# andimarafioti/faster-qwen3-tts

Measured on AMD Instinct MI355X. Metric: real-time factor (audio s / wall s), Qwen3-TTS-12Hz-0.6B voice-clone streaming chunk_size=8; p50 TTFA in ttfa_ms_p50, higher is better.
Workload: dtype bf16

## Files before the change

### faster-qwen3-tts_amd/csrc/decode_kernels.cuh

```cuda
#pragma once
#include "fq3_common.cuh"
#include <initializer_list>

namespace fq3 {

enum { PRO_PLAIN = 0, PRO_NORM = 1, PRO_COMBINE = 2 };
enum { EPI_STORE = 0, EPI_RESIDUAL = 1, EPI_SWIGLU = 2 };

constexpr int kHeadDim = 128;
constexpr int kKeysPerTile = 64;
constexpr int kMaxWorkers = 8;
constexpr int kPartStride = kHeadDim + 4;


struct GemvArgs {
    const void* W; int N; int K;
    const void* x;
    const void* norm_w; float eps;
    const void* bias;
    void* y;
    const void* res;
    void* xn_out;
    int up_off;
    const float* part; int n_part; int rep;
// ... 244 lines not shown
    const void* x = PRO == PRO_COMBINE ? static_cast<const void*>(a.part) : a.x;
    hipLaunchKernelGGL((gemv_kernel<T, NCH, PRO, EPI, NT, M, R>), dim3(grid), dim3(256), shm, s, a.W, x, a.norm_w, a.N, a.K, a.eps, a.up_off,
                       a.n_part, a.rep, t);
}

struct AttnArgs {
    const void* qkv;
    const void* q_norm_w; const void* k_norm_w; float eps;
    const float* cos_row; const float* sin_row;
    void* kcache; void* vcache; int max_seq;
    const int* table; int blk_stride;
    const int* pos_ptr; int pos_imm; int n_pad;
    const int* done_ptr;
    int n_kv; float* part; float scale;
    int rep; void* out;
};

template <typename T, int REP, bool PAGED>
__device__ __forceinline__ void attn_decode_body(const AttnArgs& a) {
    constexpr int HD = kHeadDim, KS = kKeysPerTile, NG = KS / 16;
    const int g = blockIdx.x, s = blockIdx.y, S = gridDim.y;
    __shared__ float qs[REP][HD];
    __shared__ float knew[HD], vnew[HD];
    __shared__ float wo[4][REP][HD];
    __shared__ float wm[4][REP], wl[4][REP];
    const int tid = threadIdx.x, wave = tid >> 6, lane = tid & 63;
    const int sub = lane >> 4, c = lane & 15;
    const T* qkv = reinterpret_cast<const T*>(a.qkv);
    const int q_dim = a.n_kv * REP * HD, kv_dim = a.n_kv * HD;
    T* kc = reinterpret_cast<T*>(a.kcache) + (PAGED ? (size_t)g * KS * HD : (size_t)g * a.max_seq * HD);
// ... 166 lines not shown
constexpr int kAttnDecodeLeadDwords = 14;
template <typename T, int REP, bool PAGED>
__global__ __launch_bounds__(256) void attn_decode_kernel(const int* table, const void* qkv, void* kcache, void* vcache, const int* pos_ptr,
                                                          int max_seq, int n_kv, int blk_stride, int pos_imm, AttnTail t) {
    AttnArgs a = attn_args_of(t);
    a.table = table; a.qkv = qkv; a.kcache = kcache; a.vcache = vcache; a.pos_ptr = pos_ptr;
    a.max_seq = max_seq; a.n_kv = n_kv; a.blk_stride = blk_stride; a.pos_imm = pos_imm;
    attn_decode_body<T, REP, PAGED>(a);
}
template <typename T, int REP, bool PAGED>
inline void attn_decode_launch(const AttnArgs& a, int workers, hipStream_t s) {
    hipLaunchKernelGGL((attn_decode_kernel<T, REP, PAGED>), dim3(a.n_kv, workers), dim3(256), 0, s, a.table, a.qkv, a.kcache, a.vcache, a.pos_ptr,
                       a.max_seq, a.n_kv, a.blk_stride, a.pos_imm, attn_tail(a));
}

template <typename T>
__device__ __forceinline__ void attn_pred_body(const AttnArgs& a, int head) {
    constexpr int HD = kHeadDim;
    const int g = head / a.rep, hh = head - g * a.rep;
    const int lane = threadIdx.x & 63, sub = lane >> 4, c = lane & 15;
    const int pos = a.pos_imm;
    const T* qkv = reinterpret_cast<const T*>(a.qkv);
    const int q_dim = a.n_kv * a.rep * HD, kv_dim = a.n_kv * HD;
    T* kc = reinterpret_cast<T*>(a.kcache) + (size_t)g * a.max_seq * HD;
    T* vc = reinterpret_cast<T*>(a.vcache) + (size_t)g * a.max_seq * HD;
    Raw8<T> qraw, knraw, vnraw, qwraw, kwraw, kr[4], vr[4];
    ldraw<false>(qraw, qkv + (size_t)head * HD + c * 8);
    ldraw<false>(knraw, qkv + q_dim + (size_t)g * HD + c * 8);
    ldraw<false>(vnraw, qkv + q_dim + kv_dim + (size_t)g * HD + c * 8);
    ldraw<false>(qwraw, reinterpret_cast<const T*>(a.q_norm_w) + c * 8);
    ldraw<false>(kwraw, reinterpret_cast<const T*>(a.k_norm_w) + c * 8);
    const f32x4 cs0 = *reinterpret_cast<const f32x4*>(a.cos_row + ((c * 8) & 63)), cs1 = *reinterpret_cast<const f32x4*>(a.cos_row + ((c * 8 + 4) & 63));
    const f32x4 sn0 = *reinterpret_cast<const f32x4*>(a.sin_row + ((c * 8) & 63)), sn1 = *reinterpret_cast<const f32x4*>(a.sin_row + ((c * 8 + 4) & 63));
#pragma unroll
    for (int i = 0; i < 4; ++i) {
        int key = i * 4 + sub;
        key = key < a.max_seq ? key : a.max_seq - 1;
        ldraw<false>(kr[i], kc + (size_t)key * HD + c * 8);
        ldraw<false>(vr[i], vc + (size_t)key * HD + c * 8);
    }
    __builtin_amdgcn_sched_barrier(0);
    const float sgn = c < 8 ? -1.f : 1.f;
    const float cs[8] = {cs0.x, cs0.y, cs0.z, cs0.w, cs1.x, cs1.y, cs1.z, cs1.w};
    const float sn[8] = {sgn * sn0.x, sgn * sn0.y, sgn * sn0.z, sgn * sn0.w, sgn * sn1.x, sgn * sn1.y, sgn * sn1.z, sgn * sn1.w};
    auto norm_rope = [&](const Raw8<T>& raw, const Raw8<T>& wraw, float (&out)[8]) {
#pragma clang fp contract(off)
        float x[8], w[8];
        unpack(raw, x); unpack(wraw, w);
        float ss = 0.f;
#pragma unroll
        for (int i = 0; i < 8; ++i) ss = fmaf(x[i], x[i], ss);
        ss = row16_sum(ss);
        const float rs = 1.0f / sqrtf(ss / (float)HD + a.eps);
#pragma unroll
        for (int i = 0; i < 8; i += 2) {
            float u = x[i] * rs, v = x[i + 1] * rs;
            DT<T>::rnd2(u, v);
            u *= w[i]; v *= w[i + 1];
            DT<T>::rnd2(u, v);
            x[i] = u; x[i + 1] = v;
        }
#pragma unroll
        for (int i = 0; i < 8; i += 2) {
            float a0 = x[i] * cs[i], a1 = x[i + 1] * cs[i + 1];
            float b0 = row16_xor8(x[i]) * sn[i], b1 = row16_xor8(x[i + 1]) * sn[i + 1];
            DT<T>::rnd2(a0, a1); DT<T>::rnd2(b0, b1);
            float r0 = a0 + b0, r1 = a1 + b1;
            DT<T>::rnd2(r0, r1);
            out[i] = r0; out[i + 1] = r1;
        }
    };
    float qr[8], knew[8], vnew[8];
    norm_rope(qraw, qwraw, qr);
    norm_rope(knraw, kwraw, knew);
    unpack(vnraw, vnew);
    if (hh == 0 && sub == 0) {
        DT<T>::st8(kc + (size_t)pos * HD + c * 8, knew);
        DT<T>::st8(vc + (size_t)pos * HD + c * 8, vnew);
    }
    float sc[5];
#pragma unroll
    for (int i = 0; i < 4; ++i) {
        float kf[8], s = 0.f;
        unpack(kr[i], kf);
#pragma unroll
        for (int d = 0; d < 8; ++d) s = fmaf(qr[d], kf[d], s);
        s = row16_sum(s);
        sc[i] = (i * 4 + sub < pos) ? s * a.scale : -INFINITY;
    }
    {
        float s = 0.f;
#pragma unroll
        for (int d = 0; d < 8; ++d) s = fmaf(qr[d], knew[d], s);
        s = row16_sum(s);
        sc[4] = sub == 0 ? s * a.scale : -INFINITY;
    }
    const float mx = wave_max(fmaxf(fmaxf(fmaxf(sc[0], sc[1]), fmaxf(sc[2], sc[3])), sc[4]));
    float p[5], lsum = 0.f, o[8];
#pragma unroll
    for (int i = 0; i < 5; ++i) { p[i] = __expf(sc[i] - mx); lsum += p[i]; }
    lsum = wave_sum(lsum) * (1.0f / 16.0f);
#pragma unroll
    for (int d = 0; d < 8; ++d) o[d] = p[4] * vnew[d];
#pragma unroll
    for (int i = 0; i < 4; ++i) {
        float vf[8];
        if (!(i * 4 + sub < pos)) zero(vr[i]);
        unpack(vr[i], vf);
#pragma unroll
        for (int d = 0; d < 8; ++d) o[d] = fmaf(p[i], vf[d], o[d]);
    }
    const float inv = 1.0f / lsum;
#pragma unroll
    for (int d = 0; d < 8; ++d) o[d] = xrow_sum(o[d]) * inv;
    if (sub == 0) DT<T>::st8(reinterpret_cast<T*>(a.out) + (size_t)head * HD + c * 8, o);
}

template <typename T>
__device__ __forceinline__ void attn_pred_body(const AttnArgs& a) { attn_pred_body<T>(a, (int)blockIdx.x); }

template <typename T, int REP>
__device__ __forceinline__ void attn_pred_group_body(const AttnArgs& a, int g) {
    constexpr int HD = kHeadDim;
// ... 103 lines not shown
}

constexpr int kAttnPredLeadDwords = 14;
template <typename T>
__global__ __launch_bounds__(64) void attn_pred_kernel(const void* qkv, const void* q_norm_w, const void* k_norm_w, void* kcache, void* vcache,
                                                       int n_kv, int rep, int max_seq, int pos_imm, AttnTail t) {
    AttnArgs a = attn_args_of(t);
    a.qkv = qkv; a.q_norm_w = q_norm_w; a.k_norm_w = k_norm_w; a.kcache = kcache; a.vcache = vcache;
    a.n_kv = n_kv; a.rep = rep; a.max_seq = max_seq; a.pos_imm = pos_imm;
    attn_pred_body<T>(a);
}
template <typename T>
inline void attn_pred_launch(const AttnArgs& a, int heads, hipStream_t s) {
    hipLaunchKernelGGL((attn_pred_kernel<T>), dim3(heads), dim3(64), 0, s, a.qkv, a.q_norm_w, a.k_norm_w, a.kcache, a.vcache,
                       a.n_kv, a.rep, a.max_seq, a.pos_imm, attn_tail(a));
}

template <typename T>
__global__ __launch_bounds__(256) void rmsnorm_kernel(const T* x, const T* w, T* y, int K, float eps) {
    __shared__ float red[8];
    float ss = 0.f;
    for (int e = threadIdx.x; e < K; e += 256) { const float v = DT<T>::ld(x + e); ss = fmaf(v, v, ss); }
    ss = block_sum<4>(ss, red);
    const float rs = 1.0f / sqrtf(ss / (float)K + eps);
    for (int e = threadIdx.x; e < K; e += 256)
        DT<T>::st(y + e, DT<T>::ld(w + e) * DT<T>::rnd(DT<T>::ld(x + e) * rs));
}

template <typename T>
__global__ void copy_kernel(T* dst, const T* src, int n) {
// ... 126 lines not shown
```

### faster-qwen3-tts_amd/csrc/fq3_api.hip

```cpp
#define FQ3_SKINNY_EXTERN
#include "fq3_ctx.h"
#include "sampler.cuh"
#include "sampler_wave.cuh"
#include "skinny_gemm.cuh"

#include <cstdio>
#include <cstdlib>
#include <cstring>
#include <map>
#include <string>
#include <type_traits>
#include <vector>

using namespace fq3;

static thread_local std::string g_err;
static int fail(int code, const std::string& m) { g_err = m; return code; }
int fq3_fail_(int code, const std::string& m) { return fail(code, m); }
#define HIPCHK(x) do { hipError_t e_ = (x); if (e_ != hipSuccess) return fail(FQ3_EHIP, std::string(#x) + ": " + hipGetErrorString(e_)); } while (0)

extern "C" const char* fq3_last_error(void) { return g_err.c_str(); }
extern "C" void fq3_set_error_(const char* msg) { g_err = msg ? msg : ""; }
extern "C" int fq3_abi_version(void) { return FQ3_ABI_VERSION; }

// ... 190 lines not shown
    if ((r = dmalloc(c, &c->qkv2, (size_t)qkvm * c->esz))) return r;
    if ((r = dmalloc(c, &c->attn_out, (size_t)qkvm * c->esz))) return r;
    if ((r = dmalloc(c, &c->attn_out2, (size_t)qkvm * c->esz))) return r;
    if ((r = dmalloc(c, &c->act2, (size_t)Im * c->esz))) return r;
    if ((r = dmalloc(c, &c->pred_x2, (size_t)p.hidden * c->esz))) return r;
    if ((r = dmalloc(c, &c->xin, (size_t)Hm * c->esz))) return r;
    if ((r = dmalloc(c, &c->tmp_hidden, (size_t)Hm * c->esz))) return r;
    if ((r = dmalloc(c, &c->qkv, (size_t)qkvm * c->esz))) return r;
    if ((r = dmalloc(c, &c->act, (size_t)Im * c->esz))) return r;
    if ((r = dmalloc(c, &c->logits, (size_t)Vm * c->esz))) return r;
    if ((r = dmalloc(c, &c->past_hidden, (size_t)t.hidden * c->esz))) return r;
    if ((r = dmalloc(c, &c->ph_hold, (size_t)t.hidden * c->esz))) return r;
    if ((r = dmalloc(c, &c->pred_in, (size_t)2 * t.hidden * c->esz))) return r;
    if ((r = dmalloc(c, &c->pred_next, (size_t)t.hidden * c->esz))) return r;
    if ((r = dmalloc(c, &c->pred_x, (size_t)p.hidden * c->esz))) return r;
    if ((r = dmalloc(c, &c->plogits, (size_t)(G - 1) * p.vocab * c->esz))) return r;
    const int maxkv = std::max(t.n_kv_heads, p.n_kv_heads);
    c->part_stride = (size_t)maxkv * kMaxWorkers * 4 * kPartStride;
    if ((r = dmalloc(c, (void**)&c->part, 2 * c->part_stride * sizeof(float)))) return r;
    if ((r = dmalloc(c, (void**)&c->rope_now, 2 * 64 * sizeof(float)))) return r;
    if ((r = dmalloc(c, (void**)&c->seen_api, kMaxVocab))) return r;
    if ((r = dmalloc(c, (void**)&c->st, sizeof(DecodeState)))) return r;
    if ((r = dmalloc(c, (void**)&c->seen, kMaxVocab))) return r;
    if ((r = dmalloc(c, (void**)&c->codes, (size_t)(frames + 1) * G * sizeof(int)))) return r;
    if ((r = dmalloc(c, (void**)&c->ids64, (size_t)64 * sizeof(int64_t)))) return r;
    if ((r = dmalloc(c, (void**)&c->d_pemb, (size_t)64 * sizeof(void*)))) return r;
    HIPCHK(hipStreamCreateWithFlags(&c->cap_stream, hipStreamNonBlocking));
    return FQ3_OK;
}

extern "C" int fq3_set_option(fq3_ctx* c, const char* key, int value) {
    if (!c || !key) return fail(FQ3_EINVAL, "null argument");
    const std::string k(key);
    if (k == "weight_nt") c->opt_nt = value;
    else if (k == "pred_m2") c->opt_m2 = value;
    else if (k == "pred_attn") c->opt_pred_attn = value;
    else if (k == "rows_per_wave_max") c->opt_rmax = value;
    else if (k == "prefill_mode") c->prefill_mode = value;
    else if (k == "flash_prefill") c->opt_flash_prefill = value;
    else if (k == "flash_small") c->opt_flash_small = value;
    else if (k == "cont_pack") c->opt_cont_pack = value;
    else if (k == "swiglu_tile") c->opt_swiglu_tile = value;
    else if (k == "packed_weights") c->opt_packed = value;
    else if (k == "skinny_gemm") c->opt_no_skinny = !value;
    else return fail(FQ3_EINVAL, "unknown option: " + k);
    fq3_graph_reset(c);
    return FQ3_OK;
}

extern "C" int fq3_graph_reset(fq3_ctx* c) {
    if (!c) return fail(FQ3_EINVAL, "null ctx");
    if (c->exec) { (void)hipGraphExecDestroy(c->exec); c->exec = nullptr; }
    if (c->graph) { (void)hipGraphDestroy(c->graph); c->graph = nullptr; }
    return FQ3_OK;
}

namespace {
struct PackedEntry { void* p; int refs; int N, K; };
std::mutex g_packed_mu;
// ... 14 lines not shown
        return FQ3_OK;
    }
    void* p = nullptr;
    if (hipMalloc(&p, (size_t)N * K * 2) != hipSuccess) { (void)hipGetLastError(); return fail(FQ3_ENOMEM, "no device memory for the fragment-major weight copy"); }
    skinny_pack(reinterpret_cast<const bf16_t*>(W), reinterpret_cast<bf16_t*>(p), N, K, kind == 1 ? N / 2 : (kind == 2 ? -(N / 2) : 0), nullptr);
    if (hipStreamSynchronize(nullptr) != hipSuccess) { (void)hipFree(p); return fail(FQ3_EHIP, "packing a weight matrix failed"); }
    g_packed[{W, kind}] = PackedEntry{p, 1, N, K};
    return FQ3_OK;
}
void fq3_packed_release_(const void* W, int kind) {
    std::lock_guard<std::mutex> lk(g_packed_mu);
    auto it = g_packed.find({W, kind});
    if (it == g_packed.end()) return;
    if (--it->second.refs <= 0) { (void)hipFree(it->second.p); g_packed.erase(it); }
}
static void packed_release_all(fq3_ctx* c) {
    for (auto& r : c->packed_refs) fq3_packed_release_(r.first, r.second);
    c->packed_refs.clear();
}
static int packed_acquire_all(fq3_ctx* c) {
    if (c->cfg.dtype != FQ3_BF16) return FQ3_OK;
    auto take = [&](const void* W, int N, int K, int kind) -> int {
        const int r = fq3_packed_acquire_(W, N, K, kind);
        if (r == FQ3_OK) c->packed_refs.emplace_back(W, kind);
        return r == FQ3_EUNSUPPORTED ? FQ3_OK : r;
    };
    auto stack = [&](const std::vector<fq3_layer_weights>& L, const fq3_stack_dims& d) -> int {
        const int qd = d.n_heads * kHeadDim, kvd = d.n_kv_heads * kHeadDim;
        for (const fq3_layer_weights& l : L) {
            if (int r = take(l.qkv, qd + 2 * kvd, d.hidden, 0)) return r;
            if (int r = take(l.o, d.hidden, qd, 0)) return r;
            if (int r = take(l.gate_up, 2 * d.inter, d.hidden, 1)) return r;
            if (int r = take(l.gate_up, 2 * d.inter, d.hidden, 0)) return r;
// ... 95 lines not shown
        return nt ? launch_gemv_t<bf16_t, PRO, EPI, true>(a, rmax, s) : launch_gemv_t<bf16_t, PRO, EPI, false>(a, rmax, s);
    return nt ? launch_gemv_t<float, PRO, EPI, true>(a, rmax, s) : launch_gemv_t<float, PRO, EPI, false>(a, rmax, s);
}

template <typename T, bool PAGED>
static void launch_attn_p(const AttnArgs& a, int rep, int workers, hipStream_t s) {
    with_value<1, 2, 4>(rep, [&](auto r) {
        attn_decode_launch<T, decltype(r)::value, PAGED>(a, workers, s);
    });
}
template <typename T>
static void launch_attn_t(const AttnArgs& a, int rep, int workers, hipStream_t s) {
    if (a.table) launch_attn_p<T, true>(a, rep, workers, s); else launch_attn_p<T, false>(a, rep, workers, s);
}

struct StepSrc { const void* x0; const int* pos_ptr; int pos_imm; bool kv_only_tail = false; };

static int run_stack(fq3_ctx* c, bool talker, const StepSrc& src, hipStream_t s) {
    const fq3_stack_dims& d = talker ? c->cfg.talker : c->cfg.predictor;
    const std::vector<fq3_layer_weights>& L = talker ? c->tl : c->pl;
    StackBufs& kv = talker ? c->tk : c->pk;
    const int rep = d.n_heads / d.n_kv_heads;
    const int q_dim = d.n_heads * kHeadDim, kv_dim = d.n_kv_heads * kHeadDim;
    const bool nt = c->opt_nt == 2 || (c->opt_nt == 1 && talker);
    const float *cos_row, *sin_row;
    if (src.pos_ptr) { cos_row = c->rope_now; sin_row = c->rope_now + 64; }
    else {
        const int rl = talker ? c->wt.talker_rope_len : c->wt.pred_rope_len;
        int rp = src.pos_imm + (talker ? c->rope_delta : 0);
        rp = rp < 0 ? 0 : (rp >= rl ? rl - 1 : rp);
        cos_row = (talker ? c->wt.talker_cos : c->wt.pred_cos) + (size_t)rp * 64;
        sin_row = (talker ? c->wt.talker_sin : c->wt.pred_sin) + (size_t)rp * 64;
    }
    for (int i = 0; i < d.n_layers; ++i) {
        const fq3_layer_weights& w = L[i];
        const void* xin = i == 0 ? src.x0 : c->h;
        GemvArgs g{};
        g.eps = d.rms_eps;
        g.W = w.qkv; g.N = q_dim + 2 * kv_dim; g.K = d.hidden; g.x = xin;
        g.norm_w = w.input_norm; g.y = c->qkv;
        if (int r = launch_gemv<PRO_NORM, EPI_STORE>(c, g, nt, s)) return r;
        const bool tail_skip = src.kv_only_tail && i == d.n_layers - 1;
        GemvArgs o{};
        o.W = w.o; o.N = d.hidden; o.K = q_dim; o.y = c->h; o.res = xin; o.rep = rep;
        AttnArgs a{};
        a.qkv = c->qkv; a.q_norm_w = w.q_norm; a.k_norm_w = w.k_norm; a.eps = d.rms_eps;
        a.cos_row = cos_row; a.sin_row = sin_row;
        a.kcache = kv.k[i]; a.vcache = kv.v[i]; a.max_seq = kv.max_seq;
        a.table = kv.d_table; a.blk_stride = kv.pool ? (int)kv.pool->blk_elems : 0;
        a.pos_ptr = src.pos_ptr; a.pos_imm = src.pos_imm;
        a.done_ptr = src.pos_ptr ? &c->st->done : nullptr;
        a.n_pad = talker ? c->n_pad : 0;
        a.n_kv = d.n_kv_heads; a.part = c->part;
        a.scale = 1.0f / sqrtf((float)kHeadDim);
        a.rep = rep; a.out = c->attn_out;
        const bool pred_attn = c->opt_pred_attn && !talker && !src.pos_ptr && src.pos_imm <= 16;
        if (pred_attn) {
            if (c->cfg.dtype == FQ3_BF16) attn_pred_launch<bf16_t>(a, d.n_heads, s);
            else attn_pred_launch<float>(a, d.n_heads, s);
            if (tail_skip) break;
            o.x = c->attn_out;
// ... 18 lines not shown

static int run_predictor_pair(fq3_ctx* c, const void* x_a, const void* x_b, hipStream_t s) {
    const fq3_stack_dims& d = c->cfg.predictor;
    StackBufs& kv = c->pk;
    const int rep = d.n_heads / d.n_kv_heads;
    const int q_dim = d.n_heads * kHeadDim, kv_dim = d.n_kv_heads * kHeadDim;
    for (int i = 0; i < d.n_layers; ++i) {
        const fq3_layer_weights& w = c->pl[i];
        const void* xa = i == 0 ? x_a : c->h;
        const void* xb = i == 0 ? x_b : c->h2;
        GemvArgs g{};
        g.eps = d.rms_eps; g.W = w.qkv; g.N = q_dim + 2 * kv_dim; g.K = d.hidden; g.x = xa; g.x2 = xb;
        g.norm_w = w.input_norm; g.y = c->qkv; g.y2 = c->qkv2;
        if (int r = launch_gemv2<PRO_NORM, EPI_STORE>(c, g, s)) return r;
        for (int m = 0; m < 2; ++m) {
            AttnArgs a{};
            a.qkv = m == 0 ? c->qkv : c->qkv2; a.q_norm_w = w.q_norm; a.k_norm_w = w.k_norm; a.eps = d.rms_eps;
            a.cos_row = c->wt.pred_cos + (size_t)m * 64; a.sin_row = c->wt.pred_sin + (size_t)m * 64;
            a.kcache = kv.k[i]; a.vcache = kv.v[i]; a.max_seq = kv.max_seq;
            a.pos_ptr = nullptr; a.pos_imm = m; a.n_pad = 0; a.n_kv = d.n_kv_heads;
            a.part = c->part + (size_t)m * c->part_stride; a.scale = 1.0f / sqrtf((float)kHeadDim);
            a.rep = rep; a.out = m == 0 ? c->attn_out : c->attn_out2;
            if (c->opt_pred_attn) {
                if (c->cfg.dtype == FQ3_BF16) attn_pred_launch<bf16_t>(a, d.n_heads, s);
                else attn_pred_launch<float>(a, d.n_heads, s);
            } else if (c->cfg.dtype == FQ3_BF16) launch_attn_t<bf16_t>(a, rep, kv.workers, s);
            else launch_attn_t<float>(a, rep, kv.workers, s);
        }
        GemvArgs o{};
        o.W = w.o; o.N = d.hidden; o.K = q_dim; o.y = c->h; o.y2 = c->h2; o.res = xa; o.res2 = xb; o.rep = rep;
        if (c->opt_pred_attn) {
            o.x = c->attn_out; o.x2 = c->attn_out2;
            if (int r = launch_gemv2<PRO_PLAIN, EPI_RESIDUAL>(c, o, s)) return r;
        } else {
            o.part = c->part; o.part_stride2 = c->part_stride; o.n_part = kv.workers;
            if (int r = launch_gemv2<PRO_COMBINE, EPI_RESIDUAL>(c, o, s)) return r;
        }
        GemvArgs m{};
        m.eps = d.rms_eps; m.W = w.gate_up; m.N = d.inter; m.K = d.hidden; m.x = c->h; m.x2 = c->h2;
        m.norm_w = w.post_norm; m.y = c->act; m.y2 = c->act2; m.up_off = d.inter;
        if (int r = launch_gemv2<PRO_NORM, EPI_SWIGLU>(c, m, s)) return r;
        GemvArgs dn{};
        dn.W = w.down; dn.N = d.hidden; dn.K = d.inter; dn.x = c->act; dn.x2 = c->act2; dn.y = c->h; dn.y2 = c->h2;
        dn.res = c->h; dn.res2 = c->h2;
        if (int r = launch_gemv2<PRO_PLAIN, EPI_RESIDUAL>(c, dn, s)) return r;
    }
    return 0;
}

#define NEED_BOUND(c) do { if (!(c)) return fail(FQ3_EINVAL, "null ctx"); if (!(c)->bound) return fail(FQ3_ESTATE, "weights not bound"); } while (0)
#define LAUNCH_CHECK() HIPCHK(hipGetLastError())

extern "C" int fq3_set_generation_state(fq3_ctx* c, int n_pad, int rope_delta) {
    if (!c) return fail(FQ3_EINVAL, "null ctx");
    if (n_pad < 0 || n_pad >= c->cfg.max_seq_len) return fail(FQ3_EINVAL, "n_pad out of range");
    if (c->n_pad != n_pad || c->rope_delta != rope_delta) fq3_graph_reset(c);
    c->n_pad = n_pad; c->rope_delta = rope_delta;
    return FQ3_OK;
}

template <typename T, bool TO_CACHE>
__global__ __launch_bounds__(256) void kv_paged_copy_kernel(T* cache, const int* table, int blk_stride, T* dense, int n_kv, int L) {
// ... 432 lines not shown

extern "C" int fq3_set_predictor_sampling(fq3_ctx* c, const fq3_sampling* s) {
    if (!c || !s) return fail(FQ3_EINVAL, "null argument");
    if (s->do_sample && !(s->temperature > 0.f)) return fail(FQ3_EINVAL, "temperature must be > 0");
    if ((s->top_p >= 1.0f) != (c->pred_sampling.top_p >= 1.0f)) fq3_graph_reset(c);
    c->pred_sampling = *s;
    return FQ3_OK;
}

template <typename T>
static int predictor_passes_t(fq3_ctx* c, const DecodeState* st_dev, const void* pred_input, const void* noise_imm,
                              int64_t* out64, void* out_logits, hipStream_t s) {
    const fq3_stack_dims &p = c->cfg.predictor, &t = c->cfg.talker;
    const int G = c->cfg.num_code_groups, Vp = p.vocab, Ht = t.hidden;
    SampleCfg scfg = to_cfg(c->pred_sampling);
    for (int pass = 0; pass < G; ++pass) {
        const void* hsrc = c->h;
        if (pass == 0 && c->opt_m2) {
            const T* xa = (const T*)pred_input;
            const T* xb = (const T*)pred_input + Ht;
            if (c->cfg.has_projection) {
                GemvArgs g{};
                g.W = c->wt.proj_w; g.bias = c->wt.proj_b; g.N = p.hidden; g.K = Ht; g.x = xa; g.x2 = xb; g.y = c->pred_x; g.y2 = c->pred_x2;
                if (int r = launch_gemv2<PRO_PLAIN, EPI_STORE>(c, g, s)) return r;
                xa = (const T*)c->pred_x; xb = (const T*)c->pred_x2;
            }
            if (int r = run_predictor_pair(c, xa, xb, s)) return r;
            pass = 1;
            hsrc = c->h2;
        } else {
        const T* x_talker = pass < 2 ? (const T*)pred_input + (size_t)pass * Ht : (const T*)c->pred_next;
        const void* x0 = x_talker;
        if (c->cfg.has_projection) {
            GemvArgs g{};
            g.W = c->wt.proj_w; g.bias = c->wt.proj_b; g.N = p.hidden; g.K = Ht; g.x = x_talker; g.y = c->pred_x;
            if (int r = launch_gemv<PRO_PLAIN, EPI_STORE>(c, g, false, s)) return r;
            x0 = c->pred_x;
        }
        StepSrc src{x0, nullptr, pass};
        src.kv_only_tail = pass == 0;
        if (int r = run_stack(c, false, src, s)) return r;
        }
        if (pass == 0) continue;
        const int cb = pass - 1;
        T* lg = out_logits ? (T*)out_logits + (size_t)cb * Vp : (T*)c->plogits + (size_t)cb * Vp;
        GemvArgs hgm{};
        hgm.eps = p.rms_eps; hgm.W = c->lmh[cb]; hgm.N = Vp; hgm.K = p.hidden; hgm.x = hsrc;
        hgm.norm_w = c->wt.predictor_final_norm; hgm.y = lg;
        if (int r = launch_gemv<PRO_NORM, EPI_STORE>(c, hgm, false, s)) return r;
        const T* nz = noise_imm ? (const T*)noise_imm + (size_t)cb * Vp : nullptr;
        const T* next_emb = cb + 1 < G - 1 ? (const T*)c->pemb[cb] : nullptr;
        launch_sample_pred<T>(st_dev, (const T*)lg, Vp, cb, scfg, nz, st_dev ? c->codes : nullptr, G, out64, next_emb,
                              (T*)c->pred_next, Ht, c->pred_sampling.top_p >= 1.0f, st_dev ? c->tf : nullptr, s);
    }
    return 0;
}

extern "C" int fq3_predictor_loop(fq3_ctx* c, const void* pred_input, const void* noise, int64_t* out_ids,
                                  void* out_logits, void* stream) {
    NEED_BOUND(c);
    if (!pred_input || !out_ids) return fail(FQ3_EINVAL, "null argument");
    if (c->pred_sampling.do_sample && !noise) return fail(FQ3_EINVAL, "predictor sampling enabled but no noise given");
    hipStream_t s = (hipStream_t)stream;
    int r = c->cfg.dtype == FQ3_BF16 ? predictor_passes_t<bf16_t>(c, nullptr, pred_input, noise, out_ids, out_logits, s)
                                     : predictor_passes_t<float>(c, nullptr, pred_input, noise, out_ids, out_logits, s);
    if (r) return r;
    LAUNCH_CHECK();
    return FQ3_OK;
}

__global__ __launch_bounds__(256) void decode_arm_kernel(DecodeState* st, DecodeState init, unsigned char* seen, int seen_bytes,
                                                         uint32_t* past_hidden, const uint32_t* ph_src, int ph_words) {
    for (int i = threadIdx.x; i < seen_bytes / 4; i += 256) reinterpret_cast<uint32_t*>(seen)[i] = 0u;
    for (int i = threadIdx.x; i < ph_words; i += 256) past_hidden[i] = ph_src[i];
    if (threadIdx.x == 0) *st = init;
}
__global__ void decode_set_forced_kernel(TeacherForcing* tf, const int* forced, int* decisions) {
    tf->forced = forced; tf->decisions = decisions;
// ... 74 lines not shown
    g.eps = t.rms_eps; g.W = c->wt.codec_head; g.N = t.vocab; g.K = H; g.x = c->h;
    g.norm_w = c->wt.talker_final_norm; g.y = c->logits; g.xn_out = c->past_hidden;
    if (int r = launch_gemv<PRO_NORM, EPI_STORE>(c, g, true, s)) return r;
    launch_sample_talker<T>(st, (const T*)c->logits, t.vocab, c->seen, G, c->talker_wave, c->tf, s);
    return 0;
}
static int enqueue_frame(fq3_ctx* c, hipStream_t s) {
    return c->cfg.dtype == FQ3_BF16 ? enqueue_frame_t<bf16_t>(c, s) : enqueue_frame_t<float>(c, s);
}

extern "C" int fq3_graph_capture(fq3_ctx* c, void* stream) {
    NEED_BOUND(c);
    if (c->exec) return FQ3_OK;
    (void)stream;
    hipStream_t cs = c->cap_stream;
    HIPCHK(hipStreamBeginCapture(cs, hipStreamCaptureModeRelaxed));
    int r = enqueue_frame(c, cs);
    hipGraph_t g = nullptr;
    hipError_t e = hipStreamEndCapture(cs, &g);
    if (r) { if (g) (void)hipGraphDestroy(g); return r; }
    if (e != hipSuccess) return fail(FQ3_EHIP, std::string("hipStreamEndCapture: ") + hipGetErrorString(e));
    c->graph = g;
    HIPCHK(hipGraphInstantiate(&c->exec, c->graph, nullptr, nullptr, 0));
    return FQ3_OK;
}

extern "C" int fq3_decode_frames(fq3_ctx* c, int n_frames, void* stream) {
    NEED_BOUND(c);
    hipStream_t s = (hipStream_t)stream;
    for (int i = 0; i < n_frames; ++i) {
        if (c->exec) { HIPCHK(hipGraphLaunch(c->exec, s)); }
        else if (int r = enqueue_frame(c, s)) return r;
    }
    LAUNCH_CHECK();
    return FQ3_OK;
}

extern "C" int fq3_decode_poll(fq3_ctx* c, int* n_frames_total, int* done, void* stream) {
    if (!c) return fail(FQ3_EINVAL, "null ctx");
    hipStream_t s = (hipStream_t)stream;
    DecodeState h;
    HIPCHK(hipMemcpyAsync(&h, c->st, sizeof h, hipMemcpyDeviceToHost, s));
    HIPCHK(hipStreamSynchronize(s));
    if (n_frames_total) *n_frames_total = h.frame;
// ... 20 lines not shown
```

### faster-qwen3-tts_amd/csrc/fq3_ctx.h

```cpp
#pragma once
#include "../../include/fq3hip.h"
#include "decode_kernels.cuh"
#include <hip/hip_runtime.h>
#include <mutex>
#include <string>
#include <utility>
#include <vector>

struct fq3_kv_pool {
    int dtype = 0, esz = 2, n_layers = 0, n_kv = 0, n_blocks = 0;
    size_t blk_elems = 0;
    std::vector<void*> k, v;
    std::vector<int> free_list;
    std::mutex mu;
    int in_use_high = 0;
    int users = 0;
    bool is_private = false;
};

struct StackBufs {
    std::vector<void*> k, v;
    int max_seq = 0, workers = 1;
    fq3_kv_pool* pool = nullptr;
    int* d_table = nullptr;
// ... 22 lines not shown
    fq3::TeacherForcing* tf = nullptr;
    unsigned char* seen = nullptr;
    int* codes = nullptr;
    int64_t* ids64 = nullptr;
    int n_pad = 0, rope_delta = 0;
    int opt_nt = 1;
    int opt_m2 = 1;
    int opt_pred_attn = 1;
    int opt_rmax = 2;
    int opt_flash_prefill = 1;
    int opt_flash_small = 1;
    int opt_cont_pack = 1;
    int opt_swiglu_tile = 1;
    int opt_packed = 1;
    std::vector<std::pair<const void*, int>> packed_refs;
    int opt_no_skinny = 0;
    int prefill_mode = 0;
    bool talker_wave = true;
    fq3_sampling pred_sampling{0.9f, 50, 1.0f, 1, 1.0f};
    hipGraph_t graph = nullptr;
    hipGraphExec_t exec = nullptr;
    hipStream_t cap_stream = nullptr;
    std::vector<void*> allocs;
    fq3_prompt_weights pw{};
    bool pw_bound = false;
    void *pw_x = nullptr, *pw_h = nullptr;
    int pw_cap = 0;
    void* ph_hold = nullptr;
    void *tt_tab = nullptr, *tt_x = nullptr, *tt_h = nullptr;
    int tt_alloc = 0;
// ... 25 lines not shown
```

### faster-qwen3-tts_amd/fq3hip/_lib.py

```python
from __future__ import annotations

import ctypes as C
import os

import torch

_HERE = os.path.dirname(os.path.abspath(__file__))
LIB_PATH = os.path.join(os.path.dirname(_HERE), "lib", "libfq3hip.so")

FQ3_BF16, FQ3_F32, FQ3_BF16X2 = 0, 1, 2
FQ3_PCM_F32, FQ3_PCM_S16, FQ3_PCM_MULAW, FQ3_PCM_ALAW = 0, 1, 2, 3
FQ3_OK, FQ3_EINVAL, FQ3_EHIP, FQ3_ESTATE, FQ3_ETOOLONG, FQ3_EUNSUPPORTED, FQ3_ENOMEM = 0, -1, -2, -3, -4, -5, -6

vp = C.c_void_p
i32 = C.c_int32


class StackDims(C.Structure):
    _fields_ = [("hidden", i32), ("inter", i32), ("n_layers", i32), ("n_heads", i32), ("n_kv_heads", i32),
                ("head_dim", i32), ("vocab", i32), ("rms_eps", C.c_float)]


class Config(C.Structure):
    _fields_ = [("dtype", i32), ("talker", StackDims), ("predictor", StackDims), ("num_code_groups", i32),
# ... 67 lines not shown

SIGNATURES = {
    "fq3_last_error": (C.c_char_p, []),
    "fq3_abi_version": (C.c_int, []),
    "fq3_ctx_create": (C.c_int, [C.POINTER(Config), C.POINTER(vp)]),
    "fq3_ctx_destroy": (C.c_int, [vp]),
    "fq3_kv_pool_create": (C.c_int, [C.POINTER(Config), C.c_int, C.POINTER(vp)]),
    "fq3_kv_pool_destroy": (C.c_int, [vp]),
    "fq3_kv_pool_stats": (C.c_int, [vp, C.POINTER(C.c_int), C.POINTER(C.c_int), C.POINTER(C.c_int), C.POINTER(C.c_int64)]),
    "fq3_ctx_create_pooled": (C.c_int, [C.POINTER(Config), vp, C.POINTER(vp)]),
    "fq3_kv_reserve": (C.c_int, [vp, C.c_int, vp]),
    "fq3_kv_release": (C.c_int, [vp, C.c_int]),
    "fq3_kv_blocks": (C.c_int, [vp]),
    "fq3_bind_weights": (C.c_int, [vp, C.POINTER(WeightTable)]),
    "fq3_set_option": (C.c_int, [vp, C.c_char_p, C.c_int]),
    "fq3_kv_import": (C.c_int, [vp, C.c_int, vp, vp, C.c_int, vp]),
    "fq3_kv_export": (C.c_int, [vp, C.c_int, vp, vp, C.c_int, vp]),
    "fq3_kv_adopt": (C.c_int, [vp, vp, C.c_int, vp]),
    "fq3_kv_copy": (C.c_int, [vp, vp, C.c_int, vp]),
    "fq3_set_generation_state": (C.c_int, [vp, C.c_int, C.c_int]),
    "fq3_talker_step": (C.c_int, [vp, vp, C.c_int, vp, vp]),
    "fq3_prefill": (C.c_int, [vp, vp, C.c_int, C.c_int, vp, vp, vp]),
    "fq3_prefill_continue": (C.c_int, [vp, vp, C.c_int, C.c_int, vp, vp, vp]),
    "fq3_prefill_reserve": (C.c_int, [vp]),
    "fq3_prefill_continue_batch": (C.c_int, [C.POINTER(vp), C.c_int, C.POINTER(vp), C.POINTER(C.c_int), C.POINTER(C.c_int), C.POINTER(vp),
                                             C.POINTER(vp), vp]),
    "fq3_prefill_batch": (C.c_int, [C.POINTER(vp), C.c_int, C.POINTER(vp), C.POINTER(C.c_int), C.POINTER(C.c_int), C.POINTER(vp),
                                    C.POINTER(vp), vp]),
    "fq3_set_prefill_mode": (C.c_int, [vp, C.c_int]),
    "fq3_codec_head": (C.c_int, [vp, vp, vp, vp]),
# ... 113 lines not shown
```

### faster-qwen3-tts_amd/fq3hip/engine.py

```python
from __future__ import annotations

import ctypes as C
import threading
from typing import Dict, Optional

import torch

from . import _lib as L
from .config import TTSConfig, StackConfig

Weights = Dict[str, torch.Tensor]
_CAPTURE_LOCK = threading.Lock()


def _ptr(t: Optional[torch.Tensor]) -> Optional[int]:
    return None if t is None else t.data_ptr()


def rope_tables(head_dim: int, theta: float, n_pos: int, dtype: torch.dtype):
    inv = 1.0 / (theta ** (torch.arange(0, head_dim, 2, dtype=torch.float) / head_dim))
    ang = torch.arange(n_pos, dtype=torch.float32)[:, None] * inv[None, :]
    return ang.cos().to(dtype).float().contiguous(), ang.sin().to(dtype).float().contiguous()


# ... 273 lines not shown
            e._chk(x, x.shape[0] * H, "prefill_continue embeds")
            outs.append((e.new(V), e.new(H)))
        vp = C.c_void_p
        ctxs = (vp * n)(*[e.ctx for e in engines])
        emb = (vp * n)(*[x.data_ptr() for x in embeds])
        st = (C.c_int * n)(*[int(p) for p in starts])
        cnt = (C.c_int * n)(*[int(x.shape[0]) for x in embeds])
        lg = (vp * n)(*[o[0].data_ptr() for o in outs])
        hd = (vp * n)(*[o[1].data_ptr() for o in outs])
        L.check(e0.lib.fq3_prefill_continue_batch(ctxs, n, emb, st, cnt, lg, hd, e0._stream()))
        return outs

    def set_option(self, key: str, value: int):
        L.check(self.lib.fq3_set_option(self.ctx, key.encode(), int(value)))

    def decode_set_forced(self, forced: Optional[torch.Tensor], decisions: Optional[torch.Tensor]):
        for t in (forced, decisions):
            if t is not None and (t.dtype != torch.int32 or not t.is_contiguous() or not t.is_cuda):
                raise ValueError("forced / decisions must be contiguous int32 device tensors")
        self._forced_keep = (forced, decisions)
        L.check(self.lib.fq3_decode_set_forced(self.ctx, _ptr(forced), _ptr(decisions), self._stream()))

    def set_prefill_mode(self, mode: int):
        L.check(self.lib.fq3_set_prefill_mode(self.ctx, int(mode)))

    def codec_head(self, hidden: torch.Tensor) -> torch.Tensor:
        self._chk(hidden, self.cfg.talker.hidden_size, "codec_head hidden")
        out = self.new(self.cfg.talker.vocab_size)
        L.check(self.lib.fq3_codec_head(self.ctx, hidden.data_ptr(), out.data_ptr(), self._stream()))
        return out
# ... 269 lines not shown
```

### include/fq3hip.h

```cpp
#ifndef FQ3HIP_H
#define FQ3HIP_H

#include <stdint.h>

#ifdef __cplusplus
extern "C" {
#endif

#define FQ3_ABI_VERSION 5

enum { FQ3_BF16 = 0, FQ3_F32 = 1,
       FQ3_BF16X2 = 2 };
enum { FQ3_OK = 0, FQ3_EINVAL = -1, FQ3_EHIP = -2, FQ3_ESTATE = -3, FQ3_ETOOLONG = -4, FQ3_EUNSUPPORTED = -5, FQ3_ENOMEM = -6 };

typedef struct fq3_stack_dims {
    int32_t hidden, inter, n_layers, n_heads, n_kv_heads, head_dim, vocab;
    float rms_eps;
} fq3_stack_dims;

typedef struct fq3_config {
    int32_t dtype;
    fq3_stack_dims talker;
    fq3_stack_dims predictor;
    int32_t num_code_groups;
// ... 43 lines not shown
int fq3_abi_version(void);

int fq3_ctx_create(const fq3_config* cfg, fq3_ctx** out);
int fq3_ctx_destroy(fq3_ctx* ctx);

typedef struct fq3_kv_pool fq3_kv_pool;
int fq3_kv_pool_create(const fq3_config* cfg, int n_blocks, fq3_kv_pool** out);
int fq3_kv_pool_destroy(fq3_kv_pool* pool);
int fq3_kv_pool_stats(const fq3_kv_pool* pool, int* n_blocks, int* n_free, int* high_water, int64_t* bytes_per_block);
int fq3_ctx_create_pooled(const fq3_config* cfg, fq3_kv_pool* pool, fq3_ctx** out);
int fq3_kv_reserve(fq3_ctx* ctx, int n_positions, void* stream);
int fq3_kv_release(fq3_ctx* ctx, int keep_positions);
int fq3_kv_blocks(const fq3_ctx* ctx);

int fq3_set_option(fq3_ctx* ctx, const char* key, int value);

int fq3_bind_weights(fq3_ctx* ctx, const fq3_weight_table* table);


int fq3_kv_import(fq3_ctx* ctx, int layer, const void* k, const void* v, int L, void* stream);
int fq3_kv_export(fq3_ctx* ctx, int layer, void* k, void* v, int L, void* stream);
int fq3_kv_adopt(fq3_ctx* dst, fq3_ctx* src, int L, void* stream);

int fq3_kv_copy(fq3_ctx* dst, fq3_ctx* src, int L, void* stream);

int fq3_set_generation_state(fq3_ctx* ctx, int n_pad, int rope_delta);

int fq3_talker_step(fq3_ctx* ctx, const void* embeds, int position, void* out_hidden, void* stream);

int fq3_prefill(fq3_ctx* ctx, const void* embeds, int L, int n_pad, void* out_logits, void* out_hidden,
// ... 187 lines not shown
```

Baseline: 38.95.

## Precompute predictor layer-0 QKV rows per codebook token and fuse pair attention

Builds, once per weight set, a device table holding for every predictor codebook token its projected embedding plus the layer-0 normed QKV output. The sampler writes the selected row directly, so predictor passes from the second codebook on skip the layer-0 QKV GEMV (and the projection). Separately, the first two predictor positions' attention is fused into one launch, with the second block recomputing the first position's K/V from the prior QKV instead of waiting on the cache. The cost is a large one-time table (codebooks × vocab × wide rows), a synchronous build outside graph capture, and extra memory shared across contexts.

```diff
diff --git a/faster-qwen3-tts_amd/csrc/decode_kernels.cuh b/faster-qwen3-tts_amd/csrc/decode_kernels.cuh
--- a/faster-qwen3-tts_amd/csrc/decode_kernels.cuh
+++ b/faster-qwen3-tts_amd/csrc/decode_kernels.cuh
@@ -282,6 +282,7 @@
     const int* done_ptr;
     int n_kv; float* part; float scale;
     int rep; void* out;
+    const void* qkv_prev; const float* cos_prev; const float* sin_prev;
 };
 
 template <typename T, int REP, bool PAGED>
@@ -478,12 +479,12 @@
                        a.max_seq, a.n_kv, a.blk_stride, a.pos_imm, attn_tail(a));
 }
 
-template <typename T>
+template <typename T, bool PAIR_B = false>
 __device__ __forceinline__ void attn_pred_body(const AttnArgs& a, int head) {
     constexpr int HD = kHeadDim;
     const int g = head / a.rep, hh = head - g * a.rep;
     const int lane = threadIdx.x & 63, sub = lane >> 4, c = lane & 15;
-    const int pos = a.pos_imm;
+    const int pos = PAIR_B ? 1 : a.pos_imm;
     const T* qkv = reinterpret_cast<const T*>(a.qkv);
     const int q_dim = a.n_kv * a.rep * HD, kv_dim = a.n_kv * HD;
     T* kc = reinterpret_cast<T*>(a.kcache) + (size_t)g * a.max_seq * HD;
@@ -496,6 +497,15 @@
     ldraw<false>(kwraw, reinterpret_cast<const T*>(a.k_norm_w) + c * 8);
     const f32x4 cs0 = *reinterpret_cast<const f32x4*>(a.cos_row + ((c * 8) & 63)), cs1 = *reinterpret_cast<const f32x4*>(a.cos_row + ((c * 8 + 4) & 63));
     const f32x4 sn0 = *reinterpret_cast<const f32x4*>(a.sin_row + ((c * 8) & 63)), sn1 = *reinterpret_cast<const f32x4*>(a.sin_row + ((c * 8 + 4) & 63));
+    Raw8<T> kpraw, vpraw;
+    f32x4 pc0, pc1, ps0, ps1;
+    if constexpr (PAIR_B) {
+        const T* qp = reinterpret_cast<const T*>(a.qkv_prev);
+        ldraw<false>(kpraw, qp + q_dim + (size_t)g * HD + c * 8);
+        ldraw<false>(vpraw, qp + q_dim + kv_dim + (size_t)g * HD + c * 8);
+        pc0 = *reinterpret_cast<const f32x4*>(a.cos_prev + ((c * 8) & 63)); pc1 = *reinterpret_cast<const f32x4*>(a.cos_prev + ((c * 8 + 4) & 63));
+        ps0 = *reinterpret_cast<const f32x4*>(a.sin_prev + ((c * 8) & 63)); ps1 = *reinterpret_cast<const f32x4*>(a.sin_prev + ((c * 8 + 4) & 63));
+    } else {
 #pragma unroll
     for (int i = 0; i < 4; ++i) {
         int key = i * 4 + sub;
@@ -503,11 +513,12 @@
         ldraw<false>(kr[i], kc + (size_t)key * HD + c * 8);
         ldraw<false>(vr[i], vc + (size_t)key * HD + c * 8);
     }
+    }
     __builtin_amdgcn_sched_barrier(0);
     const float sgn = c < 8 ? -1.f : 1.f;
     const float cs[8] = {cs0.x, cs0.y, cs0.z, cs0.w, cs1.x, cs1.y, cs1.z, cs1.w};
     const float sn[8] = {sgn * sn0.x, sgn * sn0.y, sgn * sn0.z, sgn * sn0.w, sgn * sn1.x, sgn * sn1.y, sgn * sn1.z, sgn * sn1.w};
-    auto norm_rope = [&](const Raw8<T>& raw, const Raw8<T>& wraw, float (&out)[8]) {
+    auto norm_rope = [&](const Raw8<T>& raw, const Raw8<T>& wraw, float (&out)[8], const float (&cs)[8], const float (&sn)[8]) {
 #pragma clang fp contract(off)
         float x[8], w[8];
         unpack(raw, x); unpack(wraw, w);
@@ -535,9 +546,16 @@
         }
     };
     float qr[8], knew[8], vnew[8];
-    norm_rope(qraw, qwraw, qr);
-    norm_rope(knraw, kwraw, knew);
+    norm_rope(qraw, qwraw, qr, cs, sn);
+    norm_rope(knraw, kwraw, knew, cs, sn);
     unpack(vnraw, vnew);
+    float kprev[8], vprev[8];
+    if constexpr (PAIR_B) {
+        const float pcs[8] = {pc0.x, pc0.y, pc0.z, pc0.w, pc1.x, pc1.y, pc1.z, pc1.w};
+        const float psn[8] = {sgn * ps0.x, sgn * ps0.y, sgn * ps0.z, sgn * ps0.w, sgn * ps1.x, sgn * ps1.y, sgn * ps1.z, sgn * ps1.w};
+        norm_rope(kpraw, kwraw, kprev, pcs, psn);
+        unpack(vpraw, vprev);
+    }
     if (hh == 0 && sub == 0) {
         DT<T>::st8(kc + (size_t)pos * HD + c * 8, knew);
         DT<T>::st8(vc + (size_t)pos * HD + c * 8, vnew);
@@ -546,7 +564,10 @@
 #pragma unroll
     for (int i = 0; i < 4; ++i) {
         float kf[8], s = 0.f;
-        unpack(kr[i], kf);
+        if constexpr (PAIR_B) {
+#pragma unroll
+            for (int d = 0; d < 8; ++d) kf[d] = i == 0 ? kprev[d] : 0.f;
+        } else unpack(kr[i], kf);
 #pragma unroll
         for (int d = 0; d < 8; ++d) s = fmaf(qr[d], kf[d], s);
         s = row16_sum(s);
@@ -569,8 +590,13 @@
 #pragma unroll
     for (int i = 0; i < 4; ++i) {
         float vf[8];
+        if constexpr (PAIR_B) {
+#pragma unroll
+            for (int d = 0; d < 8; ++d) vf[d] = (i == 0 && sub == 0) ? vprev[d] : 0.f;
+        } else {
         if (!(i * 4 + sub < pos)) zero(vr[i]);
         unpack(vr[i], vf);
+        }
 #pragma unroll
         for (int d = 0; d < 8; ++d) o[d] = fmaf(p[i], vf[d], o[d]);
     }
@@ -704,6 +730,30 @@
 inline void attn_pred_launch(const AttnArgs& a, int heads, hipStream_t s) {
     hipLaunchKernelGGL((attn_pred_kernel<T>), dim3(heads), dim3(64), 0, s, a.qkv, a.q_norm_w, a.k_norm_w, a.kcache, a.vcache,
                        a.n_kv, a.rep, a.max_seq, a.pos_imm, attn_tail(a));
+}
+
+constexpr int kAttnPredPairLeadDwords = 14;
+struct AttnPairTail { AttnTail t; void* out_b; int max_seq; };
+template <typename T>
+__global__ __launch_bounds__(64) void attn_pred_pair_kernel(const void* qkv_a, const void* qkv_b, const void* q_norm_w, const void* k_norm_w,
+                                                            void* kcache, void* vcache, int n_kv, int rep, AttnPairTail pt) {
+    AttnArgs a = attn_args_of(pt.t);
+    a.q_norm_w = q_norm_w; a.k_norm_w = k_norm_w; a.kcache = kcache; a.vcache = vcache;
+    a.n_kv = n_kv; a.rep = rep; a.max_seq = pt.max_seq;
+    if (blockIdx.y == 0) {
+        a.qkv = qkv_a; a.pos_imm = 0;
+        attn_pred_body<T>(a, (int)blockIdx.x);
+    } else {
+        a.qkv = qkv_b; a.qkv_prev = qkv_a; a.pos_imm = 1; a.out = pt.out_b;
+        a.cos_prev = a.cos_row; a.sin_prev = a.sin_row; a.cos_row += 64; a.sin_row += 64;
+        attn_pred_body<T, true>(a, (int)blockIdx.x);
+    }
+}
+template <typename T>
+inline void attn_pred_pair_launch(const AttnArgs& a, const void* qkv_b, void* out_b, int heads, hipStream_t s) {
+    const AttnPairTail pt{attn_tail(a), out_b, a.max_seq};
+    hipLaunchKernelGGL((attn_pred_pair_kernel<T>), dim3(heads, 2), dim3(64), 0, s, a.qkv, qkv_b, a.q_norm_w, a.k_norm_w, a.kcache, a.vcache,
+                       a.n_kv, a.rep, pt);
 }
 
 template <typename T>
diff --git a/faster-qwen3-tts_amd/csrc/fq3_api.hip b/faster-qwen3-tts_amd/csrc/fq3_api.hip
--- a/faster-qwen3-tts_amd/csrc/fq3_api.hip
+++ b/faster-qwen3-tts_amd/csrc/fq3_api.hip
@@ -228,6 +228,7 @@
     if ((r = dmalloc(c, &c->pred_in, (size_t)2 * t.hidden * c->esz))) return r;
     if ((r = dmalloc(c, &c->pred_next, (size_t)t.hidden * c->esz))) return r;
     if ((r = dmalloc(c, &c->pred_x, (size_t)p.hidden * c->esz))) return r;
+    if ((r = dmalloc(c, &c->pred_row, ((size_t)p.hidden + (size_t)(p.n_heads + 2 * p.n_kv_heads) * kHeadDim) * c->esz))) return r;
     if ((r = dmalloc(c, &c->plogits, (size_t)(G - 1) * p.vocab * c->esz))) return r;
     const int maxkv = std::max(t.n_kv_heads, p.n_kv_heads);
     c->part_stride = (size_t)maxkv * kMaxWorkers * 4 * kPartStride;
@@ -257,6 +258,8 @@
     else if (k == "swiglu_tile") c->opt_swiglu_tile = value;
     else if (k == "packed_weights") c->opt_packed = value;
     else if (k == "skinny_gemm") c->opt_no_skinny = !value;
+    else if (k == "pred_l0_rows") c->opt_l0_rows = value;
+    else if (k == "pred_pair_attn") c->opt_pair_attn = value;
     else return fail(FQ3_EINVAL, "unknown option: " + k);
     fq3_graph_reset(c);
     return FQ3_OK;
@@ -301,9 +304,31 @@
     if (it == g_packed.end()) return;
     if (--it->second.refs <= 0) { (void)hipFree(it->second.p); g_packed.erase(it); }
 }
+namespace {
+struct RowsEntry { void* p; int refs; size_t bytes; };
+std::map<std::vector<uintptr_t>, RowsEntry> g_rows;
+}
+static void rows_release(fq3_ctx* c) {
+    c->rows = nullptr; c->rows_failed = false;
+    if (c->rows_key.empty()) return;
+    std::lock_guard<std::mutex> lk(g_packed_mu);
+    auto it = g_rows.find(c->rows_key);
+    if (it != g_rows.end() && --it->second.refs <= 0) { (void)hipFree(it->second.p); g_rows.erase(it); }
+    c->rows_key.clear();
+}
+extern "C" int fq3_pred_rows_stats(int* n_tables, int* n_refs, int64_t* bytes) {
+    std::lock_guard<std::mutex> lk(g_packed_mu);
+    int refs = 0; int64_t b = 0;
+    for (auto& e : g_rows) { refs += e.second.refs; b += (int64_t)e.second.bytes; }
+    if (n_tables) *n_tables = (int)g_rows.size();
+    if (n_refs) *n_refs = refs;
+    if (bytes) *bytes = b;
+    return FQ3_OK;
+}
 static void packed_release_all(fq3_ctx* c) {
     for (auto& r : c->packed_refs) fq3_packed_release_(r.first, r.second);
     c->packed_refs.clear();
+    rows_release(c);
 }
 static int packed_acquire_all(fq3_ctx* c) {
     if (c->cfg.dtype != FQ3_BF16) return FQ3_OK;
@@ -429,7 +454,7 @@
     if (a.table) launch_attn_p<T, true>(a, rep, workers, s); else launch_attn_p<T, false>(a, rep, workers, s);
 }
 
-struct StepSrc { const void* x0; const int* pos_ptr; int pos_imm; bool kv_only_tail = false; };
+struct StepSrc { const void* x0; const int* pos_ptr; int pos_imm; bool kv_only_tail = false; const void* l0_qkv = nullptr; };
 
 static int run_stack(fq3_ctx* c, bool talker, const StepSrc& src, hipStream_t s) {
     const fq3_stack_dims& d = talker ? c->cfg.talker : c->cfg.predictor;
@@ -454,12 +479,13 @@
         g.eps = d.rms_eps;
         g.W = w.qkv; g.N = q_dim + 2 * kv_dim; g.K = d.hidden; g.x = xin;
         g.norm_w = w.input_norm; g.y = c->qkv;
-        if (int r = launch_gemv<PRO_NORM, EPI_STORE>(c, g, nt, s)) return r;
+        const bool have_qkv = i == 0 && src.l0_qkv;
+        if (!have_qkv) if (int r = launch_gemv<PRO_NORM, EPI_STORE>(c, g, nt, s)) return r;
         const bool tail_skip = src.kv_only_tail && i == d.n_layers - 1;
         GemvArgs o{};
         o.W = w.o; o.N = d.hidden; o.K = q_dim; o.y = c->h; o.res = xin; o.rep = rep;
         AttnArgs a{};
-        a.qkv = c->qkv; a.q_norm_w = w.q_norm; a.k_norm_w = w.k_norm; a.eps = d.rms_eps;
+        a.qkv = have_qkv ? src.l0_qkv : c->qkv; a.q_norm_w = w.q_norm; a.k_norm_w = w.k_norm; a.eps = d.rms_eps;
         a.cos_row = cos_row; a.sin_row = sin_row;
         a.kcache = kv.k[i]; a.vcache = kv.v[i]; a.max_seq = kv.max_seq;
         a.table = kv.d_table; a.blk_stride = kv.pool ? (int)kv.pool->blk_elems : 0;
@@ -508,6 +534,7 @@
         g.norm_w = w.input_norm; g.y = c->qkv; g.y2 = c->qkv2;
         if (int r = launch_gemv2<PRO_NORM, EPI_STORE>(c, g, s)) return r;
         for (int m = 0; m < 2; ++m) {
+            if (m == 1 && c->opt_pred_attn && c->opt_pair_attn) break;
             AttnArgs a{};
             a.qkv = m == 0 ? c->qkv : c->qkv2; a.q_norm_w = w.q_norm; a.k_norm_w = w.k_norm; a.eps = d.rms_eps;
             a.cos_row = c->wt.pred_cos + (size_t)m * 64; a.sin_row = c->wt.pred_sin + (size_t)m * 64;
@@ -515,7 +542,10 @@
             a.pos_ptr = nullptr; a.pos_imm = m; a.n_pad = 0; a.n_kv = d.n_kv_heads;
             a.part = c->part + (size_t)m * c->part_stride; a.scale = 1.0f / sqrtf((float)kHeadDim);
             a.rep = rep; a.out = m == 0 ? c->attn_out : c->attn_out2;
-            if (c->opt_pred_attn) {
+            if (c->opt_pred_attn && c->opt_pair_attn) {
+                if (c->cfg.dtype == FQ3_BF16) attn_pred_pair_launch<bf16_t>(a, c->qkv2, c->attn_out2, d.n_heads, s);
+                else attn_pred_pair_launch<float>(a, c->qkv2, c->attn_out2, d.n_heads, s);
+            } else if (c->opt_pred_attn) {
                 if (c->cfg.dtype == FQ3_BF16) attn_pred_launch<bf16_t>(a, d.n_heads, s);
                 else attn_pred_launch<float>(a, d.n_heads, s);
             } else if (c->cfg.dtype == FQ3_BF16) launch_attn_t<bf16_t>(a, rep, kv.workers, s);
@@ -540,6 +570,53 @@
         if (int r = launch_gemv2<PRO_PLAIN, EPI_RESIDUAL>(c, dn, s)) return r;
     }
     return 0;
+}
+
+static void rows_ensure(fq3_ctx* c, hipStream_t s) {
+    if (!c->opt_l0_rows || c->rows || c->rows_failed) return;
+    hipStreamCaptureStatus cap = hipStreamCaptureStatusNone;
+    if (hipStreamIsCapturing(s, &cap) != hipSuccess) { (void)hipGetLastError(); return; }
+    if (cap != hipStreamCaptureStatusNone) return;
+    const fq3_stack_dims &p = c->cfg.predictor, &t = c->cfg.talker;
+    const int G = c->cfg.num_code_groups, Vp = p.vocab, Ht = t.hidden, n_cb = G - 2;
+    const int qkv_n = (p.n_heads + 2 * p.n_kv_heads) * kHeadDim, Wrow = p.hidden + qkv_n;
+    if (n_cb < 1 || c->pl.empty() || (!c->cfg.has_projection && Ht != p.hidden)) { c->rows_failed = true; return; }
+    const fq3_layer_weights& l0 = c->pl[0];
+    std::vector<uintptr_t> key{(uintptr_t)l0.qkv, (uintptr_t)l0.input_norm, (uintptr_t)(c->cfg.has_projection ? c->wt.proj_w : nullptr),
+                               (uintptr_t)(c->cfg.has_projection ? c->wt.proj_b : nullptr), (uintptr_t)c->cfg.dtype, (uintptr_t)p.hidden,
+                               (uintptr_t)Ht, (uintptr_t)qkv_n, (uintptr_t)Vp, (uintptr_t)n_cb};
+    uint32_t eps_bits; memcpy(&eps_bits, &p.rms_eps, 4); key.push_back(eps_bits);
+    for (int cb = 0; cb < n_cb; ++cb) key.push_back((uintptr_t)c->pemb[cb]);
+    std::lock_guard<std::mutex> lk(g_packed_mu);
+    auto it = g_rows.find(key);
+    if (it != g_rows.end()) { ++it->second.refs; c->rows = it->second.p; c->rows_key = key; return; }
+    const size_t rowb = (size_t)Wrow * c->esz, bytes = (size_t)n_cb * Vp * rowb;
+    void* tab = nullptr;
+    if (hipMalloc(&tab, bytes) != hipSuccess) { (void)hipGetLastError(); c->rows_failed = true; return; }
+    const std::string err_keep = g_err;
+    bool ok = true;
+    const bool nt = c->opt_nt == 2;
+    for (int cb = 0; cb < n_cb && ok; ++cb) {
+        char* base = (char*)tab + (size_t)cb * Vp * rowb;
+        if (!c->cfg.has_projection)
+            ok = hipMemcpy2DAsync(base, rowb, c->pemb[cb], (size_t)Ht * c->esz, (size_t)Ht * c->esz, Vp, hipMemcpyDeviceToDevice, s) == hipSuccess;
+        for (int tok = 0; tok < Vp && ok; ++tok) {
+            char* row = base + (size_t)tok * rowb;
+            if (c->cfg.has_projection) {
+                GemvArgs g{};
+                g.W = c->wt.proj_w; g.bias = c->wt.proj_b; g.N = p.hidden; g.K = Ht; g.x = (const char*)c->pemb[cb] + (size_t)tok * Ht * c->esz; g.y = row;
+                ok = launch_gemv<PRO_PLAIN, EPI_STORE>(c, g, false, s) == 0;
+            }
+            GemvArgs g{};
+            g.eps = p.rms_eps; g.W = l0.qkv; g.N = qkv_n; g.K = p.hidden; g.x = row; g.norm_w = l0.input_norm; g.y = row + (size_t)p.hidden * c->esz;
+            ok = ok && launch_gemv<PRO_NORM, EPI_STORE>(c, g, nt, s) == 0;
+        }
+    }
+    ok = ok && hipGetLastError() == hipSuccess;
+    ok = (hipStreamSynchronize(s) == hipSuccess) && ok;
+    if (!ok) { (void)hipGetLastError(); (void)hipFree(tab); g_err = err_keep; c->rows_failed = true; return; }
+    g_rows[key] = RowsEntry{tab, 1, bytes};
+    c->rows = tab; c->rows_key = key;
 }
 
 #define NEED_BOUND(c) do { if (!(c)) return fail(FQ3_EINVAL, "null ctx"); if (!(c)->bound) return fail(FQ3_ESTATE, "weights not bound"); } while (0)
@@ -1002,6 +1079,8 @@
     const fq3_stack_dims &p = c->cfg.predictor, &t = c->cfg.talker;
     const int G = c->cfg.num_code_groups, Vp = p.vocab, Ht = t.hidden;
     SampleCfg scfg = to_cfg(c->pred_sampling);
+    const bool rows = c->opt_l0_rows && c->rows;
+    const int Wrow = p.hidden + (p.n_heads + 2 * p.n_kv_heads) * kHeadDim;
     for (int pass = 0; pass < G; ++pass) {
         const void* hsrc = c->h;
         if (pass == 0 && c->opt_m2) {
@@ -1016,6 +1095,10 @@
             if (int r = run_predictor_pair(c, xa, xb, s)) return r;
             pass = 1;
             hsrc = c->h2;
+        } else if (rows && pass >= 2) {
+            StepSrc src{c->pred_row, nullptr, pass};
+            src.l0_qkv = (const T*)c->pred_row + p.hidden;
+            if (int r = run_stack(c, false, src, s)) return r;
         } else {
         const T* x_talker = pass < 2 ? (const T*)pred_input + (size_t)pass * Ht : (const T*)c->pred_next;
         const void* x0 = x_talker;
@@ -1038,8 +1121,10 @@
         if (int r = launch_gemv<PRO_NORM, EPI_STORE>(c, hgm, false, s)) return r;
         const T* nz = noise_imm ? (const T*)noise_imm + (size_t)cb * Vp : nullptr;
         const T* next_emb = cb + 1 < G - 1 ? (const T*)c->pemb[cb] : nullptr;
+        if (rows && next_emb) next_emb = (const T*)c->rows + (size_t)cb * Vp * Wrow;
         launch_sample_pred<T>(st_dev, (const T*)lg, Vp, cb, scfg, nz, st_dev ? c->codes : nullptr, G, out64, next_emb,
-                              (T*)c->pred_next, Ht, c->pred_sampling.top_p >= 1.0f, st_dev ? c->tf : nullptr, s);
+                              rows ? (T*)c->pred_row : (T*)c->pred_next, rows ? Wrow : Ht, c->pred_sampling.top_p >= 1.0f,
+                              st_dev ? c->tf : nullptr, s);
     }
     return 0;
 }
@@ -1050,6 +1135,7 @@
     if (!pred_input || !out_ids) return fail(FQ3_EINVAL, "null argument");
     if (c->pred_sampling.do_sample && !noise) return fail(FQ3_EINVAL, "predictor sampling enabled but no noise given");
     hipStream_t s = (hipStream_t)stream;
+    rows_ensure(c, s);
     int r = c->cfg.dtype == FQ3_BF16 ? predictor_passes_t<bf16_t>(c, nullptr, pred_input, noise, out_ids, out_logits, s)
                                      : predictor_passes_t<float>(c, nullptr, pred_input, noise, out_ids, out_logits, s);
     if (r) return r;
@@ -1154,6 +1240,7 @@
     if (c->exec) return FQ3_OK;
     (void)stream;
     hipStream_t cs = c->cap_stream;
+    rows_ensure(c, cs);
     HIPCHK(hipStreamBeginCapture(cs, hipStreamCaptureModeRelaxed));
     int r = enqueue_frame(c, cs);
     hipGraph_t g = nullptr;
@@ -1168,6 +1255,7 @@
 extern "C" int fq3_decode_frames(fq3_ctx* c, int n_frames, void* stream) {
     NEED_BOUND(c);
     hipStream_t s = (hipStream_t)stream;
+    if (!c->exec && n_frames > 0) rows_ensure(c, s);
     for (int i = 0; i < n_frames; ++i) {
         if (c->exec) { HIPCHK(hipGraphLaunch(c->exec, s)); }
         else if (int r = enqueue_frame(c, s)) return r;
diff --git a/faster-qwen3-tts_amd/csrc/fq3_ctx.h b/faster-qwen3-tts_amd/csrc/fq3_ctx.h
--- a/faster-qwen3-tts_amd/csrc/fq3_ctx.h
+++ b/faster-qwen3-tts_amd/csrc/fq3_ctx.h
@@ -2,6 +2,7 @@
 #include "../../include/fq3hip.h"
 #include "decode_kernels.cuh"
 #include <hip/hip_runtime.h>
+#include <cstdint>
 #include <mutex>
 #include <string>
 #include <utility>
@@ -60,6 +61,12 @@
     int opt_swiglu_tile = 1;
     int opt_packed = 1;
     std::vector<std::pair<const void*, int>> packed_refs;
+    int opt_l0_rows = 1;
+    int opt_pair_attn = 1;
+    void* pred_row = nullptr;
+    const void* rows = nullptr;
+    bool rows_failed = false;
+    std::vector<uintptr_t> rows_key;
     int opt_no_skinny = 0;
     int prefill_mode = 0;
     bool talker_wave = true;
diff --git a/faster-qwen3-tts_amd/fq3hip/_lib.py b/faster-qwen3-tts_amd/fq3hip/_lib.py
--- a/faster-qwen3-tts_amd/fq3hip/_lib.py
+++ b/faster-qwen3-tts_amd/fq3hip/_lib.py
@@ -105,6 +105,7 @@
     "fq3_kv_blocks": (C.c_int, [vp]),
     "fq3_bind_weights": (C.c_int, [vp, C.POINTER(WeightTable)]),
     "fq3_set_option": (C.c_int, [vp, C.c_char_p, C.c_int]),
+    "fq3_pred_rows_stats": (C.c_int, [C.POINTER(C.c_int), C.POINTER(C.c_int), C.POINTER(C.c_int64)]),
     "fq3_kv_import": (C.c_int, [vp, C.c_int, vp, vp, C.c_int, vp]),
     "fq3_kv_export": (C.c_int, [vp, C.c_int, vp, vp, C.c_int, vp]),
     "fq3_kv_adopt": (C.c_int, [vp, vp, C.c_int, vp]),
diff --git a/faster-qwen3-tts_amd/fq3hip/engine.py b/faster-qwen3-tts_amd/fq3hip/engine.py
--- a/faster-qwen3-tts_amd/fq3hip/engine.py
+++ b/faster-qwen3-tts_amd/fq3hip/engine.py
@@ -311,6 +311,11 @@
     def set_option(self, key: str, value: int):
         L.check(self.lib.fq3_set_option(self.ctx, key.encode(), int(value)))
 
+    def pred_rows_stats(self):
+        n, r, b = C.c_int(0), C.c_int(0), C.c_int64(0)
+        L.check(self.lib.fq3_pred_rows_stats(C.byref(n), C.byref(r), C.byref(b)))
+        return n.value, r.value, b.value
+
     def decode_set_forced(self, forced: Optional[torch.Tensor], decisions: Optional[torch.Tensor]):
         for t in (forced, decisions):
             if t is not None and (t.dtype != torch.int32 or not t.is_contiguous() or not t.is_cuda):
diff --git a/include/fq3hip.h b/include/fq3hip.h
--- a/include/fq3hip.h
+++ b/include/fq3hip.h
@@ -81,6 +81,7 @@
 int fq3_kv_blocks(const fq3_ctx* ctx);
 
 int fq3_set_option(fq3_ctx* ctx, const char* key, int value);
+int fq3_pred_rows_stats(int* n_tables, int* n_refs, int64_t* bytes);
 
 int fq3_bind_weights(fq3_ctx* ctx, const fq3_weight_table* table);
 
```

Result: faster. 39.69, median of 6 (+1.9%).
